# LuletterSoul/RP-Style-Transfer

Hardware: AMD Instinct MI355X
Metric: stylized images/sec at 512×512, 1/2/4/8 MI355X; % HBM roofline (higher is better)
Workload: dtype fp32

## Files before the change

include/rpst.h:

```cpp
#ifndef RPST_H_
#define RPST_H_

#include <stddef.h>
#include <stdint.h>

#ifdef __cplusplus
extern "C" {
#endif

typedef void* rpst_stream_t;

#define RPST_OK 0
#define RPST_EINVAL (-1)
#define RPST_EHIP (-2)
#define RPST_EWORKSPACE (-3)

#define RPST_PAD_ZERO 0
#define RPST_PAD_REFLECT 1
#define RPST_IN_NONE 0
#define RPST_IN_MAXPOOL2 1
#define RPST_IN_UPSAMPLE2 2
#define RPST_IN_ADD_UPSAMPLE2 3
#define RPST_IN_ADAIN 4
#define RPST_IN_ADD_ADAIN 5
// ... 95 lines not shown
                          size_t workspace_bytes, rpst_stream_t stream);
int rpst_ld4_fuse(const float* y, const float* fine, const float* coarse,
                  const float* params_fine, const float* params_coarse, float* out, int N,
                  int Ca, int hidden, int H, int W, int h, int w, rpst_stream_t stream);

int rpst_conv2d_skip_adain(const float* stylized, const float* content, const float* params,
                           const float* packed_weight, const float* bias, float* out, int N,
                           int Cin, int H, int W, int Cout, int ksize, int pad_mode, int relu,
                           rpst_stream_t stream);

int64_t rpst_conv2d_grid_threads(int N, int Cin, int Hs, int Ws, int Cout, int ksize,
                                 int in_op);

#define RPST_CONV_DIRECT 0
#define RPST_CONV_WINOGRAD 1
#define RPST_CONV_WINOGRAD4 2
#define RPST_CONV_NARROW 3
int rpst_conv2d_algorithm(int Cout, int Cin, int Hs, int Ws, int ksize, int in_op);

int rpst_conv2d_set_precise(int on);

int rpst_conv2d_set_quarter(int mode);
int rpst_conv2d_quarter(int Cout, int Cin, int Hs, int Ws, int ksize, int in_op);

int rpst_maxpool2x2_ceil(const float* in, float* out, int N, int C, int H, int W,
                         rpst_stream_t stream);
int rpst_upsample_nearest2x(const float* in, float* out, int N, int C, int H, int W,
                            rpst_stream_t stream);
int rpst_add_upsample_nearest2x(const float* a, const float* b, float* out, int N, int C, int H,
                                int W, rpst_stream_t stream);

size_t rpst_sanet_attention_workspace_size(int B, int HW);
size_t rpst_sanet_attention_workspace_size_c(int B, int C, int HW);
int rpst_sanet_attention(const float* F, const float* G, const float* H, float* O, int B,
                         int C, int HW, void* workspace, size_t workspace_bytes,
                         rpst_stream_t stream);

size_t rpst_cosine_affinity_workspace_size(int B, int C, int HW);
int rpst_cosine_affinity(const float* content, const float* style, float* out, int B, int C,
                         int HW, void* workspace, size_t workspace_bytes, rpst_stream_t stream);

size_t rpst_aea_clamp_workspace_size(int B, int HW, int hidden);
int rpst_aea_clamp(const float* x, const float* fx, const float* w1, const float* b1,
                   const float* w2, const float* b2, int hidden, int mode, float scale,
                   float from, float interval, float* out_fx, float* out_clamp, int B, int HW,
                   void* workspace, size_t workspace_bytes, rpst_stream_t stream);
// ... 134 lines not shown
```

rp-style-transfer_amd/csrc/rpst_conv.h:

```cpp
#pragma once

#include "rpst_common.h"

namespace rpst {

constexpr int kTW = 32;

struct ConvArgs {
  const float* in;
  const float* aux;
  const float* aux2;
  const float* wpk;
  const float* bias;
  const float* res;
  float* out;
  int N, Cin, Hs, Ws, H, W, Cout, Cout_pad, nchunks;
  int tiles_x, tiles_y, co_tiles;
  int pad, relu;
  int persist;
  int cosplit;
  float2* stat_part;
  int stat_P;
  int64_t wstride;
  const float* btab;
  int skip_from;
  const float* in2;
  int in2_from;
  const float* mask;
  int pool_out;
};

struct ConvMode {
  int precise;
  int quarter;
  int algo;
  bool narrow;
  int narrow_rpt;
};

struct ConvTiling {
  int64_t blocks;
  int nth;
  int stat_nt, stat_wn, stat_tw;
  bool stat_t;
};

__device__ __forceinline__ const float* conv_in_img(const ConvArgs& a, int n, int64_t per) {
  return (a.in2_from > 0 && n >= a.in2_from) ? a.in2 + (int64_t)(n - a.in2_from) * per
                                             : a.in + (int64_t)n * per;
}

template <int KS>
struct ConvK {
  static constexpr int CK = (KS == 3) ? 8 : 16;
  static constexpr int TAPS = KS * KS;
  static constexpr int KCH = TAPS * CK;
};
// ... 222 lines not shown
```

rp-style-transfer_amd/csrc/rpst_conv.hip:

```cpp
#include "rpst_conv.h"

#include <cstdlib>
#include <cstring>

namespace rpst {

template <int KS, int BM, int TH, int WM, int WN, int INOP, int NTH, int CKK, bool DB,
          bool GATED = false>
__global__ __launch_bounds__(NTH, 2) void conv_mfma_kernel(ConvArgs a) {
  using K = ConvK<KS>;
  constexpr int PCK = K::CK, TAPS = K::TAPS;
  constexpr int CK = CKK, KCH = TAPS * CK;
  static_assert(PCK % CK == 0, "kernel chunk must divide the packing chunk");
  constexpr int OFF = (KS == 3) ? 1 : 0;
  constexpr int PH = TH + KS - 1, PW = kTW + KS - 1;
  constexpr int WTM = BM / WM;
  constexpr int MT = WTM / 32;
  constexpr int NT = TH / WN;
  static_assert(WM * WN == NTH / kWave, "one wave per sub-tile");
  static_assert(MT >= 1 && NT >= 1 && (CK % 2) == 0, "tile");
  constexpr int NW4 = KCH * BM / 4;
  constexpr int WLD = (NW4 + NTH - 1) / NTH;
  constexpr bool WFULL = (NW4 % NTH) == 0;
  constexpr int GROUPS = NTH / 32;
// ... 532 lines not shown
  a.tiles_x = (a.W + kTW - 1) / kTW;
  a.tiles_y = (a.H + th - 1) / th;
  a.co_tiles = a.Cout_pad / bm;
  a.stat_P = a.tiles_x * a.tiles_y * wn;
  return {(int64_t)a.tiles_x * a.tiles_y * a.N * a.co_tiles, 256, th / wn, wn, kTW, false};
}

static int narrow_rpt(int Cout, const ConvMode& m) {
  return Cout <= 4 && m.narrow_rpt != 2 ? 4 : 2;
}
static ConvTiling narrow_tiling(ConvArgs& a, int rpt) {
  const int rows = 4 * rpt;
  a.Cout_pad = pad_cout(a.Cout);
  a.nchunks = (a.Cin + ConvK<3>::CK - 1) / ConvK<3>::CK;
  a.tiles_x = (a.W + kNrTW - 1) / kNrTW;
  a.tiles_y = (a.H + rows - 1) / rows;
  a.co_tiles = 1;
  a.stat_P = 0;
  return {(int64_t)a.tiles_x * a.tiles_y * a.N, 256, 0, 0, kNrTW, false};
}

static thread_local int t_conv_precise = 0;
static thread_local int t_conv_quarter = -1;

static ConvMode conv_mode() {
  ConvMode m{};
  m.precise = t_conv_precise;
  const char* e = getenv("RPST_W4Q");
  const int q = t_conv_quarter >= 0 ? t_conv_quarter : ((e && *e) ? atoi(e) : 1);
  m.quarter = q == 2 ? 2 : q != 0;
  e = getenv("RPST_CONV_ALGO");
  m.algo = -1;
  if (e && e[0] == 'd') m.algo = RPST_CONV_DIRECT;
  else if (e && !strcmp(e, "winograd")) m.algo = RPST_CONV_WINOGRAD;
  else if (e && !strcmp(e, "winograd4")) m.algo = RPST_CONV_WINOGRAD4;
  e = getenv("RPST_CONV_NARROW");
  m.narrow = !(e && *e && atoi(e) == 0);
  e = getenv("RPST_CONV_NARROW_RPT");
  m.narrow_rpt = (e && *e && atoi(e) == 2) ? 2 : 0;
  return m;
}

static int conv_algo(int Cout, int Cin, int Hs, int Ws, int ksize, int in_op, const ConvMode& m) {
  if (ksize != 3) return RPST_CONV_DIRECT;
  const bool w4 = wino4_supports(in_op) && wino4_fits(1, Cin, Hs, Ws, in_op);
  const bool nr = (in_op == RPST_IN_NONE || (in_op == RPST_IN_ADD_ADAIN && Cout <= 4)) &&
                  narrow_shape(Cin, Cout) && m.narrow;
  if (m.algo == RPST_CONV_DIRECT) return nr ? RPST_CONV_NARROW : RPST_CONV_DIRECT;
  if (m.algo == RPST_CONV_WINOGRAD) return RPST_CONV_WINOGRAD;
  if (m.algo == RPST_CONV_WINOGRAD4) return w4 ? RPST_CONV_WINOGRAD4 : RPST_CONV_WINOGRAD;
  if (nr) return RPST_CONV_NARROW;
  if (Cin <= 4 && w4 && m.precise != 1) return RPST_CONV_WINOGRAD4;
  if (Cin < 16) return RPST_CONV_DIRECT;
// ... 38 lines not shown
  int rpt;
  size_t wofs;
  bool tall;
  ConvTiling t;
};

static ConvPlan conv_plan(ConvArgs& a, int ksize, int in_op, const ConvMode& m, ConvNeeds need) {
  ConvPlan p{};
  p.op = in_op;
  p.algo = conv_algo(a.Cout, a.Cin, a.Hs, a.Ws, ksize, in_op, m);
  if (p.algo == RPST_CONV_NARROW) {
    p.rpt = narrow_rpt(a.Cout, m);
    p.t = narrow_tiling(a, p.rpt);
    if (need.stats || a.N > 65535 || a.tiles_y > 65535) p.algo = RPST_CONV_DIRECT;
  }
  if (need.residual && (p.algo == RPST_CONV_WINOGRAD || p.algo == RPST_CONV_WINOGRAD4))
    p.algo = RPST_CONV_DIRECT;
  if (p.algo == RPST_CONV_WINOGRAD4) {
    p.fold = need.fold && !need.stats && a.H >= 2 && a.W >= 2;
    if (p.fold) p.op = RPST_IN_NONE;
    p.quarter = wino4q_applies(a.Cin, a.Cout, p.op, m);
    p.wofs = direct_packed_floats(a.Cout, a.Cin, ksize) + wino_packed_floats(a.Cout, a.Cin) +
             (p.quarter ? wino4_packed_floats(a.Cout, a.Cin) : 0);
    p.t = p.quarter ? wino4q_tiling(a) : wino4_tiling(a);
  } else if (p.algo == RPST_CONV_WINOGRAD) {
    p.wofs = direct_packed_floats(a.Cout, a.Cin, ksize);
    p.t = wino_tiling(a, in_op);
  } else if (p.algo == RPST_CONV_DIRECT) {
    p.tall = need.gated && need.stats && direct_bm(a.Cout) != 128;
    p.t = direct_tiling(a, ksize, in_op, p.tall);
  }
  return p;
}

template <class F>
static size_t max_over_modes(ConvMode m, F bytes) {
  size_t best = 0;
  for (m.precise = 0; m.precise < 3; ++m.precise)
    for (m.quarter = 0; m.quarter < 3; ++m.quarter) {
      const size_t b = bytes(m);
      best = b > best ? b : best;
    }
  return best;
}

}
// ... 11 lines not shown

static ConvPlan query_plan(int N, int Cin, int Hs, int Ws, int Cout, int ksize, int in_op) {
  ConvArgs a = conv_shape(N, Cin, Hs, Ws, Cout, in_op);
  return conv_plan(a, ksize, in_op, conv_mode(), {});
}

extern "C" int64_t rpst_conv2d_grid_threads(int N, int Cin, int Hs, int Ws, int Cout,
                                            int ksize, int in_op) {
  if (N <= 0 || Cin <= 0 || Hs <= 0 || Ws <= 0 || Cout <= 0 || (ksize != 1 && ksize != 3))
    return 0;
  const ConvTiling t = query_plan(N, Cin, Hs, Ws, Cout, ksize, in_op).t;
  return t.blocks * t.nth;
}

extern "C" int rpst_conv2d_set_precise(int on) {
  const int old = t_conv_precise;
  t_conv_precise = on == 2 ? 2 : on != 0;
  return old;
}

extern "C" int rpst_conv2d_set_quarter(int mode) {
  const int old = t_conv_quarter;
  t_conv_quarter = mode < 0 ? -1 : (mode > 2 ? 2 : mode);
  return old;
}

extern "C" int rpst_conv2d_algorithm(int Cout, int Cin, int Hs, int Ws, int ksize, int in_op) {
  return query_plan(1, Cin, Hs, Ws, Cout, ksize, in_op).algo;
}

extern "C" int rpst_conv2d_quarter(int Cout, int Cin, int Hs, int Ws, int ksize, int in_op) {
  return query_plan(1, Cin, Hs, Ws, Cout, ksize, in_op).quarter ? 1 : 0;
}

extern "C" int rpst_conv2d_pack(const float* weight, float* packed, int Cout, int Cin,
                                int ksize, rpst_stream_t stream) {
  RPST_REQUIRE(weight && packed, "conv2d_pack: null pointer");
  RPST_REQUIRE(Cout > 0 && Cin > 0, "conv2d_pack: bad channels");
  RPST_REQUIRE(ksize == 1 || ksize == 3, "conv2d_pack: ksize must be 1 or 3, got %d", ksize);
  const int64_t total = (int64_t)direct_packed_floats(Cout, Cin, ksize);
  const int threads = 256;
  conv_pack_kernel<<<(unsigned)((total + threads - 1) / threads), threads, 0,
                     as_stream(stream)>>>(weight, packed, Cout, Cin, ksize, ck_of(ksize),
                                          pad_cout(Cout), total);
  if (int e = launch_status("conv_pack_kernel")) return e;
  if (ksize == 3) {
// ... 522 lines not shown
```

rp-style-transfer_amd/csrc/rpst_wino4q.hip:

```cpp
#include "rpst_conv.h"

#include <type_traits>

#ifndef RPST_W4Q_DBG
#define RPST_W4Q_DBG 0
#endif

namespace rpst {
namespace {

template <int PAD>
__device__ __forceinline__ void q_mfma(floatx4& acc, float a, float b) {
  if constexpr (PAD)
    asm volatile("s_nop 1\n\tv_mfma_f32_16x16x4_f32 %0, %1, %2, %0" : "+v"(acc) : "v"(a), "v"(b));
  else
    asm volatile("v_mfma_f32_16x16x4_f32 %0, %1, %2, %0" : "+v"(acc) : "v"(a), "v"(b));
}
__device__ __forceinline__ unsigned q_lds_addr(const float* p) {
  return (unsigned)(uintptr_t)(const __attribute__((address_space(3))) float*)p;
}
template <int OFF>
__device__ __forceinline__ void q_dma16(__amdgpu_buffer_rsrc_t r, unsigned m0, unsigned voff,
                                        int soff) {
  asm volatile("s_mov_b32 m0, %0\n\ts_nop 0\n\tbuffer_load_dwordx4 %1, %2, %3 offen offset:%4 lds"
// ... 24 lines not shown
    u2 = fmaf(4.f, d1, fmaf(-5.f, d3, d5));
  }
}

}

constexpr int kQCo = 64;
constexpr int kQTH = 8, kQTW = 64;
constexpr int kQXO = 4;
constexpr int kQPS = 72;
constexpr int kQCS = 768;
constexpr int kQWS = 9216;
constexpr int kQPAT = 4 * kQCS;
constexpr int kQNTH = 512;
constexpr int kQMaxCo = 512;
constexpr int kQWPI = 5;
constexpr int kQWide = 2, kQSlow = 6;
constexpr int kQDMA4 = 3, kQDMA = 12;
constexpr int kQRP = kQPS / 4;
constexpr int kQXS = 4 * 3 * 3 * 64 * 2;
constexpr int kQWG0 = 0;
constexpr int kQPG = 5;
constexpr int kQAhead = 3;
static_assert(10 * kQRP <= kQDMA4 * 64 && kQDMA4 * 256 <= kQCS, "16-B pieces in a channel");
static_assert(10 * kQPS <= kQDMA * 64 && kQDMA * 64 <= kQCS, "4-B pieces in a channel");
static_assert(2 * kQWide >= kQDMA4 && 2 * kQSlow >= kQDMA && 8 * kQWPI >= 36, "coverage");
static_assert(2 * kQXS <= kQWS, "the exchange fits a weight stage");
static_assert((2 * kQWS + 4 * kQPAT) * 4 + 1024 + kQSlow * kQNTH * 4 + 9 * kQMaxCo * 4 <= 163840,
              "LDS");

template <typename TW>
__global__ void wino4q_pack_kernel(const TW* __restrict__ w, float* __restrict__ pk, int Cout,
                                   int Cin, int K4, int64_t per, int64_t total, int64_t sco,
                                   int64_t sci, int64_t stap) {
  int64_t t = (int64_t)blockIdx.x * blockDim.x + threadIdx.x;
  if (t >= total) return;
  const int64_t img = t / per;
  pk += img * per;
  w += img * (int64_t)Cout * Cin * 9;
  t -= img * per;
  const int cb = (int)(t & 3);
  int64_t r = t >> 2;
  const int l = (int)(r & 63);
  r >>= 6;
  const int p = (int)(r % 9);
  r /= 9;
// ... 53 lines not shown
  const int ci = ks * 4 + (l >> 4);
  const int64_t nc = (int64_t)N * Cin, i = (int64_t)n * Cin + (ci < Cin ? ci : 0);
  const float sc = ci < Cin ? aux[3 * nc + i] / aux[2 * nc + i] : 0.f;
  const float4 v = pk[u];
  out[t] = make_float4(v.x * sc, v.y * sc, v.z * sc, v.w * sc);
}

int wino4q_fold_w(const float* pk, float* out, const float* aux, int N, int Cout, int Cin,
                  hipStream_t st) {
  const int64_t per4 = (int64_t)wino4q_packed_floats(Cout, Cin) / 4, n4 = (int64_t)N * per4;
  wino4q_fold_w_kernel<<<(unsigned)((n4 + 255) / 256), 256, 0, st>>>(
      reinterpret_cast<const float4*>(pk), reinterpret_cast<float4*>(out), aux, N, Cin,
      (Cin + 3) / 4, per4);
  return launch_status("wino4q_fold_w_kernel");
}

bool wino4q_applies(int Cin, int Cout, int in_op, const ConvMode& m) {
  const int min_cin = m.quarter == 2 ? 16 : 128;
  return m.quarter && m.precise != 2 && (in_op == RPST_IN_NONE || in_op == RPST_IN_UPSAMPLE2) &&
         Cout >= 64 && Cout <= kQMaxCo &&
         Cin >= min_cin && Cin % 16 == 0;
}

ConvTiling wino4q_tiling(ConvArgs& a) {
  a.Cout_pad = (a.Cout + kQCo - 1) / kQCo * kQCo;
  a.nchunks = (a.Cin + 3) / 4;
  a.tiles_x = (a.W + kQTW - 1) / kQTW;
  a.tiles_y = (a.H + kQTH - 1) / kQTH;
  a.co_tiles = a.Cout_pad / kQCo;
  a.stat_P = a.tiles_x * a.tiles_y * 2;
  a.cosplit = 1;
  return {(int64_t)a.tiles_x * a.tiles_y * a.N, kQNTH, 4, kQTH / 4, kQTW, true};
}

struct QEpi {
  int W, H, Cout, gy0, gx0, rows, n, sidx;
  bool vec, full, bst, edge, store, pool;
  float inv, slope;
  unsigned voff[4];
  float* out;
  float* oimg;
  unsigned obytes;
  const float* btab;
  float2* statp;
  int statP;
};

__device__ __forceinline__ QEpi q_epi_ctx(int wr, int tn) {
  const KArgs L = late_args();
  QEpi e;
  e.W = L->W;
  e.H = L->H;
  e.Cout = L->Cout;
  e.slope = L->relu == RPST_ACT_RELU ? 0.f : (L->relu == RPST_ACT_LRELU ? 0.2f : 1.f);
  int btx, bty;
  w4_tile((int)blockIdx.x / L->cosplit, L->tiles_x, L->tiles_y, btx, bty, e.n);
  const int bx0 = btx * kQTW;
  e.gy0 = bty * kQTH + 4 * wr;
  e.gx0 = bx0 + 4 * tn;
  e.vec = (e.W & 3) == 0 && e.gx0 + 3 < e.W;
  e.rows = max(0, min(4, e.H - e.gy0));
  const int cols = max(0, min(kQTW, e.W - bx0));
  e.inv = e.rows * cols > 0 ? __builtin_amdgcn_rcpf((float)(e.rows * cols)) : 0.f;
  e.full = e.rows == 4 && bx0 + kQTW <= e.W;
  e.edge = e.gy0 == 0 || e.gy0 + 4 >= e.H || bx0 == 0 || bx0 + kQTW >= e.W;
  e.out = L->out;
  const int64_t plane = (int64_t)e.H * e.W;
  e.pool = L->pool_out != 0;
  e.bst = !e.pool && (e.W & 3) == 0 && (int64_t)e.Cout * plane * 4 < (1LL << 31);
  e.oimg = e.out + (int64_t)e.n * e.Cout * plane;
  const bool keep = L->skip_from <= 0 || e.n < L->skip_from;
  e.obytes = keep ? (unsigned)(e.Cout * plane * 4) : 0u;
  e.store = keep;
#pragma unroll
  for (int yy = 0; yy < 4; ++yy)
    e.voff[yy] = (yy < e.rows && e.gx0 < e.W) ? (unsigned)(((e.gy0 + yy) * e.W + e.gx0) * 4)
                                             : 0x80000000u;
  e.btab = L->btab;
  e.statp = L->stat_part;
// ... 120 lines not shown
  }
}

template <int INOP, bool STATS, bool BTAB, bool RELU>
__global__ __launch_bounds__(kQNTH, 1) void wino4q_mfma_kernel(ConvArgs a) {
  __shared__ __attribute__((aligned(16))) float ws0[kQWS];
  __shared__ __attribute__((aligned(16))) float ws1[kQWS];
  __shared__ __attribute__((aligned(16))) float ps0[kQPAT];
  __shared__ __attribute__((aligned(16))) float ps1[kQPAT];
  __shared__ __attribute__((aligned(16))) float ps2[kQPAT];
  __shared__ __attribute__((aligned(16))) float ps3[kQPAT];
  __shared__ __attribute__((aligned(16))) float dummy[256];
  __shared__ unsigned poffs[kQSlow][kQNTH];
  __shared__ float btl[BTAB ? 9 * kQMaxCo : kQMaxCo];

  const int wave = __builtin_amdgcn_readfirstlane((int)threadIdx.x >> 6);
  const int lane = threadIdx.x & 63;
  const int k = lane >> 4, tn = lane & 15, wr = wave >> 2;

  int bid = (int)blockIdx.x;
  const int cog = bid % a.cosplit;
  bid /= a.cosplit;
  const int nct = a.co_tiles / a.cosplit, ct0 = cog * nct;
  int tx, ty, n;
  w4_tile(bid, a.tiles_x, a.tiles_y, tx, ty, n);
  const int K4 = a.nchunks, G = nct * K4;
  const int y0 = ty * kQTH, x0 = tx * kQTW;

  {
    const int nb = BTAB ? 9 * a.Cout : a.Cout;
    const float* src = BTAB ? a.btab + (int64_t)n * nb : a.bias;
    for (int i = threadIdx.x; i < nb; i += kQNTH) btl[i] = src ? src[i] : 0.f;
  }
  constexpr bool up = INOP == RPST_IN_UPSAMPLE2;
  const unsigned in_plane = up ? (unsigned)(a.Hs * a.Ws) : (unsigned)(a.H * a.W);
  const unsigned oob = a.Cin * in_plane * 4u;
  const float* in_img = conv_in_img(a, n, (int64_t)a.Cin * in_plane);
  const unsigned wbytes = (unsigned)(nct * K4 * kQWS) * 4u;
  const float* w_img = a.wpk + (int64_t)n * a.wstride + (int64_t)ct0 * K4 * kQWS;

  const int hf = wave & 1;
  const bool zp = a.pad == RPST_PAD_ZERO;
  const int rs = up ? a.Ws : a.W;
  const bool w4a = (a.W & 3) == 0;
  const bool wide = !up && ((x0 >= 1 && x0 + kQTW < a.W) || (w4a && x0 + kQTW <= a.W));
  const bool fixL = wide && w4a && !zp && x0 == 0;
  const bool fixR = wide && w4a && !zp && x0 + kQTW == a.W;
  unsigned poff[kQSlow];
  const int tid = threadIdx.x;
  if (wide) {
#pragma unroll
    for (int i = 0; i < kQWide; ++i) {
      const int p = kQWide * hf + i;
      const int f = 64 * p + lane, row = min(f / kQRP, 9), j = f - (f / kQRP) * kQRP;
      int y = y0 - 1 + row;
      const int xs = x0 - kQXO + 4 * j;
      const bool okx = !w4a || (xs >= 0 && xs + 3 < a.W);
      const bool ok = p < kQDMA4 && f < 10 * kQRP && resolve_bf(y, a.H, zp) && okx;
      poff[i] = ok ? ((unsigned)(y * rs) + (unsigned)xs) * 4u : oob;
    }
#pragma unroll
    for (int i = kQWide; i < kQSlow; ++i) poff[i] = oob;
  } else {
#pragma unroll
    for (int i = 0; i < kQSlow; ++i) {
      const int p = kQSlow * hf + i;
      const int f = 64 * p + lane;
      const int row = min(f / kQPS, 9), col = f - (f / kQPS) * kQPS;
      int y = y0 - 1 + row, x = x0 - kQXO + col;
      const bool oky = resolve_bf(y, a.H, zp), okx = resolve_bf(x, a.W, zp);
      const bool ok = p < kQDMA && col >= kQXO - 1 && col < kQXO + 1 + kQTW &&
                      f < 10 * kQPS && oky && okx;
      poff[i] = ok ? ((unsigned)((up ? y >> 1 : y) * rs) + (unsigned)(up ? x >> 1 : x)) * 4u : oob;
    }
  }
#pragma unroll
  for (int i = 0; i < kQSlow; ++i) poffs[i][tid] = poff[i];

  constexpr int DBG = RPST_W4Q_DBG;
  const int wl = wave * 4096;
  const bool real4 = wave < 4;
  const int w4 = 32768 + wave * 1024;
  const unsigned dummy_a = q_lds_addr(dummy);
  int wso = wl;
  auto issue_w = [&](bool live, unsigned stg, auto Ic) {
    constexpr int I = decltype(Ic)::value;
    if (DBG & 2) return;
    if constexpr (I < 4) {
      q_dma16<1024 * I>(rsrc_or_zero(w_img, wbytes, live), stg + wl, lane * 16, wso);
    } else {
      q_dma16<0>(rsrc_or_zero(w_img, wbytes, live && real4), real4 ? stg + w4 : dummy_a,
                 lane * 16, wso + (w4 - wl));
    }
  };
  const unsigned pstep = 4u * in_plane * 4u;
  const int pbase = (int)((unsigned)(wave >> 1) * in_plane * 4u);
  const bool h1 = (wave & 1) != 0;
  const int pl = (wave >> 1) * (kQCS * 4) + (h1 ? (wide ? 2048 : kQSlow * 256) : 0);
  int pso = pbase;
  auto issue_p = [&](auto WIDEc, bool live, unsigned stg) {
    constexpr bool WIDE = decltype(WIDEc)::value;
    if (DBG & 1) return;
    const auto r = rsrc_or_zero(in_img, oob, live);
    const unsigned xs = stg + launder(pl);
    if constexpr (WIDE) {
      q_dma16<0>(r, xs, poffs[0][tid], pso);
      q_dma16<0>(r, h1 ? dummy_a : xs + 1024, poffs[1][tid], pso);
    } else {
#pragma unroll
      for (int i = 0; i < kQSlow; ++i) q_dma4(r, xs + 256 * i, poffs[i][tid], pso);
    }
    pso += (int)pstep;
  };
  const bool bst_all = !a.pool_out && (a.W & 3) == 0 &&
                       (int64_t)a.Cout * a.H * a.W * 4 < (1LL << 31);
  bool post_epi = false;
  auto wait_ring = [&](bool first) {
    if (DBG & 128) return;
    if (first && post_epi && bst_all) {
      if (wide) asm volatile("s_waitcnt vmcnt(18)" ::: "memory");
      else asm volatile("s_waitcnt vmcnt(22)" ::: "memory");
    } else if (wide) {
      asm volatile("s_waitcnt vmcnt(2)" ::: "memory");
    } else {
      asm volatile("s_waitcnt vmcnt(6)" ::: "memory");
    }
    if (first) post_epi = false;
  };

  auto fix_halo = [&](float* stg) {
    if ((wave == 0 && fixL) || (wave == 1 && fixR)) {
      int l = lane;
      asm volatile("" : "+v"(l));
      if (l < 40) {
        const int ch = l / 10, row = l - 10 * ch;
        float* rp = stg + ch * kQCS + row * kQPS;
        if (wave == 0) rp[kQXO - 1] = rp[kQXO + 1];
        else rp[kQXO + kQTW] = rp[kQXO + kQTW - 2];
      }
    }
  };
  auto prologue = [&](auto WIDEc) {
    issue_p(WIDEc, true, q_lds_addr(ps0));
    issue_p(WIDEc, true, q_lds_addr(ps1));
    issue_w(true, q_lds_addr(ws0), std::integral_constant<int, 0>{});
    issue_w(true, q_lds_addr(ws0), std::integral_constant<int, 1>{});
    issue_w(true, q_lds_addr(ws0), std::integral_constant<int, 2>{});
    issue_w(true, q_lds_addr(ws0), std::integral_constant<int, 3>{});
    issue_w(true, q_lds_addr(ws0), std::integral_constant<int, 4>{});
    issue_p(WIDEc, true, q_lds_addr(ps2));
    issue_p(WIDEc, true, q_lds_addr(ps3));
  };
  if (wide) prologue(std::true_type{});
  else prologue(std::false_type{});
  wait_ring(false);
  q_lds_barrier();
  if (fixL || fixR) {
    fix_halo(ps0);
    fix_halo(ps1);
    q_lds_barrier();
  }

  auto body = [&](auto Qc) {
    constexpr int Q = decltype(Qc)::value, QR = Q >> 1, QC = Q & 1;
    floatx4 acc[9][4];
#pragma unroll
    for (int p = 0; p < 9; ++p)
#pragma unroll
      for (int cb = 0; cb < 4; ++cb) acc[p][cb] = floatx4{0.f, 0.f, 0.f, 0.f};
    const int roff = k * kQCS + (4 * wr + QR) * kQPS + 4 * tn;
    auto read_row = [&](const float* stg, int rr, float (&d)[8]) {
      const float* rp = stg + roff + rr * kQPS;
      floatx4 u = *reinterpret_cast<const floatx4*>(rp + 4);
      const float e = QC ? rp[8] : rp[3];
      asm("" : "+v"(u));
      d[0] = QC ? 0.f : e; d[1] = u[0]; d[2] = u[1]; d[3] = u[2]; d[4] = u[3];
      d[5] = QC ? e : 0.f; d[6] = 0.f; d[7] = 0.f;
    };
    auto col_pass = [&](const float (&d)[8], float (&u)[3]) {
      if (DBG & 8) {
        u[0] = d[0]; u[1] = d[1]; u[2] = d[2];
        return;
      }
      q_bt3<QC>(d[0], d[1], d[2], d[3], d[4], d[5], u[0], u[1], u[2]);
    };
    auto row_pass = [&](const float (&u)[5][3], int j, float (&v)[9]) {
      if (DBG & 8) {
        v[j] = u[0][j]; v[3 + j] = u[2][j]; v[6 + j] = u[4][j];
        return;
      }
      if constexpr (QR == 0)
        q_bt3<0>(u[0][j], u[1][j], u[2][j], u[3][j], u[4][j], 0.f, v[j], v[3 + j], v[6 + j]);
      else
        q_bt3<1>(0.f, u[0][j], u[1][j], u[2][j], u[3][j], u[4][j], v[j], v[3 + j], v[6 + j]);
    };
    float V[9];
    {
      float u[5][3];
#pragma unroll
      for (int rr = 0; rr < 5; ++rr) {
        float d[8];
        read_row(ps0, rr, d);
        col_pass(d, u[rr]);
      }
#pragma unroll
      for (int j = 0; j < 3; ++j) row_pass(u, j, V);
    }

    const int woff = Q * 9 * 256 + lane * 4;
    int x = 0;
    auto step = [&](float* wsx, float* psn, float* wsn, float* psx, float* pfx, int ks,
                    bool first) {
      wait_ring(first);
      const bool wlive = x + 1 < G, plive = x + 4 < G;
      wso += kQWS * 4;
      if (first && ks + 4 == K4) pso = pbase;
      const unsigned wsn_a = q_lds_addr(wsn), psx_a = q_lds_addr(psx);
      if (DBG & 16) asm volatile("s_waitcnt lgkmcnt(0)" ::: "memory");
      else q_lds_barrier();
      constexpr int ord[9] = {0, 3, 6, 1, 4, 7, 2, 5, 8};
      constexpr int kA = kQAhead;
      float4 w4[9];
#pragma unroll
      for (int q = 0; q < kA; ++q)
        w4[ord[q]] = *reinterpret_cast<const float4*>(wsx + woff + ord[q] * 256);
      float d[8];
      read_row(psn, 0, d);
      float u[5][3];
#pragma unroll
      for (int q = 0; q < 9; ++q) {
// ... 3 lines not shown
        q_mfma<1>(acc[p][0], w4[p].x, V[p]);
        q_mfma<0>(acc[p][1], w4[p].y, V[p]);
        q_mfma<0>(acc[p][2], w4[p].z, V[p]);
        q_mfma<0>(acc[p][3], w4[p].w, V[p]);
        if (q == kQWG0) issue_w(wlive, wsn_a, std::integral_constant<int, 0>{});
        if (q == kQWG0 + 1) issue_w(wlive, wsn_a, std::integral_constant<int, 1>{});
        if (q == kQWG0 + 2) issue_w(wlive, wsn_a, std::integral_constant<int, 2>{});
        if (q == kQWG0 + 3) issue_w(wlive, wsn_a, std::integral_constant<int, 3>{});
        if (q == kQWG0 + 4) issue_w(wlive, wsn_a, std::integral_constant<int, 4>{});
        if (q == kQPG) {
          if (wide) issue_p(std::true_type{}, plive, psx_a);
          else issue_p(std::false_type{}, plive, psx_a);
        }
        if (q < 5) {
          col_pass(d, u[q]);
          if (q + 1 < 5) read_row(psn, q + 1, d);
        }
        if (q == 5 || q == 6 || q == 8) row_pass(u, q == 8 ? 2 : q - 5, V);
        if (q == 7) fix_halo(pfx);
      }
      ++x;
    };

    auto epilogue = [&](int ctile) {
      if (DBG & 32) {
        float t = 0.f;
#pragma unroll
        for (int p = 0; p < 9; ++p)
#pragma unroll
          for (int cb = 0; cb < 4; ++cb) t += acc[p][cb][0];
        if (t == 1.2345f) late_args()->out[threadIdx.x] = t;
#pragma unroll
        for (int p = 0; p < 9; ++p)
#pragma unroll
          for (int cb = 0; cb < 4; ++cb) acc[p][cb] = floatx4{0.f, 0.f, 0.f, 0.f};
        return;
      }
      q_lds_barrier();
      asm volatile("s_nop 7\n\ts_nop 4" : "+v"(acc[0][0]), "+v"(acc[0][1]), "+v"(acc[0][2]),
                   "+v"(acc[0][3]), "+v"(acc[1][0]), "+v"(acc[1][1]), "+v"(acc[1][2]),
                   "+v"(acc[1][3]), "+v"(acc[2][0]), "+v"(acc[2][1]), "+v"(acc[2][2]),
                   "+v"(acc[2][3]), "+v"(acc[3][0]), "+v"(acc[3][1]), "+v"(acc[3][2]),
                   "+v"(acc[3][3]), "+v"(acc[4][0]), "+v"(acc[4][1]));
      asm volatile("" : "+v"(acc[4][2]), "+v"(acc[4][3]), "+v"(acc[5][0]), "+v"(acc[5][1]),
                   "+v"(acc[5][2]), "+v"(acc[5][3]), "+v"(acc[6][0]), "+v"(acc[6][1]),
                   "+v"(acc[6][2]), "+v"(acc[6][3]), "+v"(acc[7][0]), "+v"(acc[7][1]),
                   "+v"(acc[7][2]), "+v"(acc[7][3]), "+v"(acc[8][0]), "+v"(acc[8][1]),
                   "+v"(acc[8][2]), "+v"(acc[8][3]));
      const int co0 = ctile * kQCo + 16 * Q + 4 * k;
#pragma unroll
      for (int rp = 0; rp < 2; ++rp) {
        float P[2][6][4];
#pragma unroll
        for (int pt = 0; pt < 3; ++pt) {
          float* xb = ws1 + wr * kQXS;
#pragma unroll
          for (int dq = 0; dq < 4; ++dq) {
            if (dq == Q || (DBG & 4)) continue;
            const int slot = (Q - dq - 1) & 3;
#pragma unroll
            for (int j = 0; j < 3; ++j)
// ... 8 lines not shown
            for (int j = 0; j < 3; ++j) {
              float2 v;
              if (s == Q || (DBG & 4)) {
                const int src = (DBG & 4) ? s : Q;
                v = make_float2(acc[3 * pt + j][src][2 * rp], acc[3 * pt + j][src][2 * rp + 1]);
              } else {
                v = *reinterpret_cast<const float2*>(
                    xb + (((Q * 3 + ((s - Q - 1) & 3)) * 3 + j) * 64 + lane) * 2);
              }
              m[0][s >> 1][3 * (s & 1) + j] = v.x;
              m[1][s >> 1][3 * (s & 1) + j] = v.y;
            }
          }
#pragma unroll
          for (int e2 = 0; e2 < 2; ++e2) {
            at6(m[e2][0], P[e2][pt]);
            at6(m[e2][1], P[e2][3 + pt]);
          }
          if (!(DBG & 4) && (rp == 0 || pt < 2)) q_lds_barrier();
        }
#pragma unroll
        for (int e2 = 0; e2 < 2; ++e2) {
          const int r = 2 * rp + e2;
          QEpi e = q_epi_ctx(wr, tn);
          e.btab = btl;
          float bias = 0.f;
          {
            const int co = co0 + r;
            if (co < e.Cout) bias = BTAB ? btl[co * 9 + 4] : btl[co];
          }
#pragma unroll
          for (int x = 0; x < 4; ++x) P[e2][1][x] += bias;
          float Y[16];
#pragma unroll
          for (int x = 0; x < 4; ++x) {
            float c6[6], y[4];
#pragma unroll
            for (int I = 0; I < 6; ++I) c6[I] = P[e2][I][x];
            at6(c6, y);
#pragma unroll
            for (int yy = 0; yy < 4; ++yy) Y[yy * 4 + x] = y[yy];
          }
          q_finish<STATS, BTAB, RELU>(e, co0 + r, Y, tn);
        }
      }
#pragma unroll
      for (int p = 0; p < 9; ++p)
#pragma unroll
        for (int cb = 0; cb < 4; ++cb) acc[p][cb] = floatx4{0.f, 0.f, 0.f, 0.f};
    };

    int ks = 0, ct = ct0;
    for (int g = 0; g < G; g += 4) {
      step(ws0, ps1, ws1, ps0, ps2, ks, true);
      step(ws1, ps2, ws0, ps1, ps3, ks + 1, false);
      step(ws0, ps3, ws1, ps2, ps0, ks + 2, false);
      step(ws1, ps0, ws0, ps3, ps1, ks + 3, false);
      ks += 4;
      if (ks == K4) {
        epilogue(ct);
        post_epi = true;
        ks = 0;
        ++ct;
      }
    }
  };
  switch (wave & 3) {
    case 0: body(std::integral_constant<int, 0>{}); break;
    case 1: body(std::integral_constant<int, 1>{}); break;
    case 2: body(std::integral_constant<int, 2>{}); break;
    default: body(std::integral_constant<int, 3>{}); break;
  }
  asm volatile("s_waitcnt vmcnt(0)" ::: "memory");
}

int wino4q_launch(ConvArgs& a, int in_op, hipStream_t st) {
  RPST_REQUIRE(in_op == RPST_IN_NONE || in_op == RPST_IN_UPSAMPLE2,
               "conv2d: winograd4 (quarter) does not support in_op %d", in_op);
  const ConvTiling t = wino4q_tiling(a);
  RPST_REQUIRE((int64_t)a.co_tiles * a.nchunks * kQWS * 4 < (1LL << 31),
               "conv2d: winograd4 weight image exceeds 2 GiB");
  RPST_REQUIRE(t.blocks <= 0x7fffffffLL, "conv2d: grid too large");
  const unsigned nb = (unsigned)t.blocks;
  const bool stats = a.stat_part != nullptr, btab = a.btab != nullptr;
  RPST_REQUIRE(!btab || in_op == RPST_IN_NONE, "conv2d: winograd4 bias table with a loader op");
  RPST_REQUIRE(!(stats && btab), "conv2d: winograd4 folded bias with statistics");
#define RPST_W4Q_GO(OP, S, B)                                                  \
  do {                                                                         \
    if (a.relu == RPST_ACT_RELU)                                               \
      wino4q_mfma_kernel<OP, S, B, true><<<nb, kQNTH, 0, st>>>(a);             \
    else                                                                       \
      wino4q_mfma_kernel<OP, S, B, false><<<nb, kQNTH, 0, st>>>(a);            \
  } while (0)
  if (in_op == RPST_IN_UPSAMPLE2) {
    if (stats) RPST_W4Q_GO(RPST_IN_UPSAMPLE2, true, false);
    else RPST_W4Q_GO(RPST_IN_UPSAMPLE2, false, false);
  } else {
// ... 10 lines not shown
```

rp-style-transfer_amd/rpst/_lib.py:

```python
from __future__ import annotations

import ctypes
import os
import threading

_HERE = os.path.dirname(os.path.abspath(__file__))
LIB_PATH = os.environ.get("RPST_LIB", os.path.join(os.path.dirname(_HERE), "csrc", "librpst.so"))

_c_float_p = ctypes.c_void_p
_P = ctypes.c_void_p
_I = ctypes.c_int
_I64 = ctypes.c_int64
_F = ctypes.c_float
_D = ctypes.c_double
_SZ = ctypes.c_size_t

SIGNATURES = {
    "rpst_version": (_I, []),
    "rpst_last_error": (ctypes.c_char_p, []),
    "rpst_calc_mean_std": (_I, [_P, _P, _P, _I, _I, _I64, _F, _P]),
    "rpst_adain_workspace_size": (_SZ, [_I, _I]),
    "rpst_adain": (_I, [_P, _P, _P, _I, _I, _I64, _F, _P, _SZ, _P]),
    "rpst_mean_variance_norm": (_I, [_P, _P, _I, _I, _I64, _F, _P, _SZ, _P]),
    "rpst_segment_plan": (_I, [_P, _P, _I, _I64, _I64, _P, _P]),
    "rpst_masked_adain_workspace_size": (_SZ, [_I, _I]),
    "rpst_masked_adain_params": (_I, [_P, _P, _P, _P, _P, _I, _I, _I64, _I64, _F, _P, _P, _SZ,
                                      _P]),
    "rpst_masked_adain_apply": (_I, [_P, _P, _P, _P, _P, _I, _I, _I64, _P]),
    "rpst_conv2d_packed_size": (_SZ, [_I, _I, _I]),
    "rpst_conv2d_pack": (_I, [_P, _P, _I, _I, _I, _P]),
    "rpst_conv2d_grid_threads": (_I64, [_I, _I, _I, _I, _I, _I, _I]),
    "rpst_conv2d_algorithm": (_I, [_I, _I, _I, _I, _I, _I]),
    "rpst_conv2d_set_precise": (_I, [_I]),
    "rpst_conv2d_set_quarter": (_I, [_I]),
    "rpst_conv2d_quarter": (_I, [_I, _I, _I, _I, _I, _I]),
    "rpst_conv2d_stats_workspace_size": (_SZ, [_I, _I, _I, _I, _I, _I, _I]),
    "rpst_conv2d_stats": (_I, [_P, _P, _P, _P, _P, _P, _I, _I, _I, _I, _I, _I, _I, _I, _I,
                               _P, _P, _F, _P, _SZ, _P]),
    "rpst_conv2d_stats_store": (_I, [_P, _P, _P, _P, _P, _P, _I, _I, _I, _I, _I, _I, _I, _I,
                                     _I, _P, _P, _F, _I, _P, _SZ, _P]),
    "rpst_conv2d": (_I, [_P, _P, _P, _P, _P, _P, _I, _I, _I, _I, _I, _I, _I, _I, _I, _P]),
    "rpst_conv2d_pool": (_I, [_P, _P, _P, _P, _P, _I, _I, _I, _I, _I, _I, _I, _I, _I, _P]),
    "rpst_conv2d_masked": (_I, [_P, _P, _P, _P, _P, _I, _I, _I, _I, _I, _I, _I, _P]),
    "rpst_conv2d_pair": (_I, [_P, _P, _I, _P, _P, _P, _I, _I, _I, _I, _I, _I, _I, _I, _P]),
    "rpst_conv2d_workspace_size": (_SZ, [_I, _I, _I, _I, _I, _I, _I]),
    "rpst_conv2d_ws": (_I, [_P, _P, _P, _P, _P, _P, _I, _I, _I, _I, _I, _I, _I, _I, _I,
                            _P, _SZ, _P]),
    "rpst_conv2d_skip_adain": (_I, [_P, _P, _P, _P, _P, _P, _I, _I, _I, _I, _I, _I, _I, _I, _P]),
    "rpst_se_gate": (_I, [_P, _P, _P, _P, _P, _P, _I, _I, _I, _P]),
    "rpst_conv2d_gated_workspace_size": (_SZ, [_I, _I, _I, _I, _I, _I]),
    "rpst_conv2d_gated": (_I, [_P, _P, _P, _P, _P, _P, _I, _I, _I, _I, _I, _I, _P, _P, _F, _P,
                               _SZ, _P]),
    "rpst_conv7_packed_size": (_SZ, [_I, _I]),
    "rpst_conv7_pack": (_I, [_P, _P, _I, _I, _P]),
    "rpst_conv7": (_I, [_P, _P, _P, _P, _P, _I, _I, _I, _I, _I, _I, _I, _I, _I, _P]),
    "rpst_nearest_index_table": (_I, [_I, _I, _P]),
    "rpst_resize_nearest": (_I, [_P, _P, _I, _I, _I, _I, _I, _I, _I, _I, _P]),
# ... 109 lines not shown
```

Before: 570.1.

## Process multiple spatial tiles per block in quarter-Winograd conv with prefetched next tile

The quarter-precision Winograd-4 conv kernel now has each block walk several consecutive output tiles instead of one. The next tile's input and weight DMA prologue is issued during the current tile's epilogue, so global loads overlap the output writes. By default a heuristic picks 2 tiles per block when the reduction is short and there are enough tiles, otherwise 1; an env var or setter can override it. This cuts launch and prologue cost and hides tile-start latency, at the price of fewer blocks (less parallelism) and more complex synchronisation through hand-tuned vmcnt waits. A debug timestamp path is also added behind a compile flag.

```diff
diff --git a/include/rpst.h b/include/rpst.h
--- a/include/rpst.h
+++ b/include/rpst.h
@@ -141,6 +141,8 @@
 
 int rpst_conv2d_set_quarter(int mode);
 int rpst_conv2d_quarter(int Cout, int Cin, int Hs, int Ws, int ksize, int in_op);
+
+int rpst_conv2d_set_tiles(int tiles);
 
 int rpst_maxpool2x2_ceil(const float* in, float* out, int N, int C, int H, int W,
                          rpst_stream_t stream);
diff --git a/rp-style-transfer_amd/csrc/rpst_conv.h b/rp-style-transfer_amd/csrc/rpst_conv.h
--- a/rp-style-transfer_amd/csrc/rpst_conv.h
+++ b/rp-style-transfer_amd/csrc/rpst_conv.h
@@ -28,11 +28,13 @@
   int in2_from;
   const float* mask;
   int pool_out;
+  int wtiles;
 };
 
 struct ConvMode {
   int precise;
   int quarter;
+  int tiles;
   int algo;
   bool narrow;
   int narrow_rpt;
diff --git a/rp-style-transfer_amd/csrc/rpst_conv.hip b/rp-style-transfer_amd/csrc/rpst_conv.hip
--- a/rp-style-transfer_amd/csrc/rpst_conv.hip
+++ b/rp-style-transfer_amd/csrc/rpst_conv.hip
@@ -578,6 +578,7 @@
 
 static thread_local int t_conv_precise = 0;
 static thread_local int t_conv_quarter = -1;
+static thread_local int t_conv_tiles = -1;
 
 static ConvMode conv_mode() {
   ConvMode m{};
@@ -585,6 +586,8 @@
   const char* e = getenv("RPST_W4Q");
   const int q = t_conv_quarter >= 0 ? t_conv_quarter : ((e && *e) ? atoi(e) : 1);
   m.quarter = q == 2 ? 2 : q != 0;
+  e = getenv("RPST_W4Q_TILES");
+  m.tiles = t_conv_tiles > 0 ? t_conv_tiles : ((e && *e) ? atoi(e) : -1);
   e = getenv("RPST_CONV_ALGO");
   m.algo = -1;
   if (e && e[0] == 'd') m.algo = RPST_CONV_DIRECT;
@@ -669,6 +672,7 @@
     p.quarter = wino4q_applies(a.Cin, a.Cout, p.op, m);
     p.wofs = direct_packed_floats(a.Cout, a.Cin, ksize) + wino_packed_floats(a.Cout, a.Cin) +
              (p.quarter ? wino4_packed_floats(a.Cout, a.Cin) : 0);
+    a.wtiles = m.tiles;
     p.t = p.quarter ? wino4q_tiling(a) : wino4_tiling(a);
   } else if (p.algo == RPST_CONV_WINOGRAD) {
     p.wofs = direct_packed_floats(a.Cout, a.Cin, ksize);
@@ -726,6 +730,12 @@
 extern "C" int rpst_conv2d_set_quarter(int mode) {
   const int old = t_conv_quarter;
   t_conv_quarter = mode < 0 ? -1 : (mode > 2 ? 2 : mode);
+  return old;
+}
+
+extern "C" int rpst_conv2d_set_tiles(int tiles) {
+  const int old = t_conv_tiles;
+  t_conv_tiles = tiles <= 0 ? -1 : tiles;
   return old;
 }
 
diff --git a/rp-style-transfer_amd/csrc/rpst_wino4q.hip b/rp-style-transfer_amd/csrc/rpst_wino4q.hip
--- a/rp-style-transfer_amd/csrc/rpst_wino4q.hip
+++ b/rp-style-transfer_amd/csrc/rpst_wino4q.hip
@@ -70,6 +70,11 @@
 constexpr int kQWG0 = 0;
 constexpr int kQPG = 5;
 constexpr int kQAhead = 3;
+constexpr int kQMaxTiles = 64;
+#if RPST_W4Q_DBG & 256
+constexpr int kQStampBlocks = 1 << 16;
+__device__ unsigned long long g_w4q_stamps[kQStampBlocks * 8];
+#endif
 static_assert(10 * kQRP <= kQDMA4 * 64 && kQDMA4 * 256 <= kQCS, "16-B pieces in a channel");
 static_assert(10 * kQPS <= kQDMA * 64 && kQDMA * 64 <= kQCS, "4-B pieces in a channel");
 static_assert(2 * kQWide >= kQDMA4 && 2 * kQSlow >= kQDMA && 8 * kQWPI >= 36, "coverage");
@@ -169,6 +174,11 @@
          Cin >= min_cin && Cin % 16 == 0;
 }
 
+static int wino4q_tiles_rule(int steps, int64_t tiles) {
+  const int t = steps <= 32 ? 2 : 1;
+  return tiles >= (int64_t)2 * 256 * t ? t : 1;
+}
+
 ConvTiling wino4q_tiling(ConvArgs& a) {
   a.Cout_pad = (a.Cout + kQCo - 1) / kQCo * kQCo;
   a.nchunks = (a.Cin + 3) / 4;
@@ -177,7 +187,10 @@
   a.co_tiles = a.Cout_pad / kQCo;
   a.stat_P = a.tiles_x * a.tiles_y * 2;
   a.cosplit = 1;
-  return {(int64_t)a.tiles_x * a.tiles_y * a.N, kQNTH, 4, kQTH / 4, kQTW, true};
+  const int64_t tiles = (int64_t)a.tiles_x * a.tiles_y * a.N;
+  if (a.wtiles <= 0) a.wtiles = wino4q_tiles_rule(a.co_tiles * a.nchunks, tiles);
+  a.wtiles = a.wtiles > kQMaxTiles ? kQMaxTiles : a.wtiles;
+  return {(tiles + a.wtiles - 1) / a.wtiles, kQNTH, 4, kQTH / 4, kQTW, true};
 }
 
 struct QEpi {
@@ -193,7 +206,7 @@
   int statP;
 };
 
-__device__ __forceinline__ QEpi q_epi_ctx(int wr, int tn) {
+__device__ __forceinline__ QEpi q_epi_ctx(int wr, int tn, int tile) {
   const KArgs L = late_args();
   QEpi e;
   e.W = L->W;
@@ -201,7 +214,7 @@
   e.Cout = L->Cout;
   e.slope = L->relu == RPST_ACT_RELU ? 0.f : (L->relu == RPST_ACT_LRELU ? 0.2f : 1.f);
   int btx, bty;
-  w4_tile((int)blockIdx.x / L->cosplit, L->tiles_x, L->tiles_y, btx, bty, e.n);
+  w4_tile(tile, L->tiles_x, L->tiles_y, btx, bty, e.n);
   const int bx0 = btx * kQTW;
   e.gy0 = bty * kQTH + 4 * wr;
   e.gx0 = bx0 + 4 * tn;
@@ -368,67 +381,94 @@
   const int cog = bid % a.cosplit;
   bid /= a.cosplit;
   const int nct = a.co_tiles / a.cosplit, ct0 = cog * nct;
-  int tx, ty, n;
-  w4_tile(bid, a.tiles_x, a.tiles_y, tx, ty, n);
   const int K4 = a.nchunks, G = nct * K4;
-  const int y0 = ty * kQTH, x0 = tx * kQTW;
-
-  {
-    const int nb = BTAB ? 9 * a.Cout : a.Cout;
-    const float* src = BTAB ? a.btab + (int64_t)n * nb : a.bias;
+  int tile = bid * a.wtiles;
+  const int ntile = min(a.wtiles, a.tiles_x * a.tiles_y * a.N - tile);
+
+  auto fill_btl = [&](int t, auto L) __attribute__((always_inline)) {
+    const int n = t / (L->tiles_x * L->tiles_y);
+    const int nb = BTAB ? 9 * L->Cout : L->Cout;
+    const float* src = BTAB ? L->btab + (int64_t)n * nb : L->bias;
     for (int i = threadIdx.x; i < nb; i += kQNTH) btl[i] = src ? src[i] : 0.f;
-  }
+  };
   constexpr bool up = INOP == RPST_IN_UPSAMPLE2;
   const unsigned in_plane = up ? (unsigned)(a.Hs * a.Ws) : (unsigned)(a.H * a.W);
   const unsigned oob = a.Cin * in_plane * 4u;
-  const float* in_img = conv_in_img(a, n, (int64_t)a.Cin * in_plane);
   const unsigned wbytes = (unsigned)(nct * K4 * kQWS) * 4u;
-  const float* w_img = a.wpk + (int64_t)n * a.wstride + (int64_t)ct0 * K4 * kQWS;
 
   const int hf = wave & 1;
-  const bool zp = a.pad == RPST_PAD_ZERO;
-  const int rs = up ? a.Ws : a.W;
-  const bool w4a = (a.W & 3) == 0;
-  const bool wide = !up && ((x0 >= 1 && x0 + kQTW < a.W) || (w4a && x0 + kQTW <= a.W));
-  const bool fixL = wide && w4a && !zp && x0 == 0;
-  const bool fixR = wide && w4a && !zp && x0 + kQTW == a.W;
-  unsigned poff[kQSlow];
   const int tid = threadIdx.x;
-  if (wide) {
-#pragma unroll
-    for (int i = 0; i < kQWide; ++i) {
-      const int p = kQWide * hf + i;
-      const int f = 64 * p + lane, row = min(f / kQRP, 9), j = f - (f / kQRP) * kQRP;
-      int y = y0 - 1 + row;
-      const int xs = x0 - kQXO + 4 * j;
-      const bool okx = !w4a || (xs >= 0 && xs + 3 < a.W);
-      const bool ok = p < kQDMA4 && f < 10 * kQRP && resolve_bf(y, a.H, zp) && okx;
-      poff[i] = ok ? ((unsigned)(y * rs) + (unsigned)xs) * 4u : oob;
-    }
-#pragma unroll
-    for (int i = kQWide; i < kQSlow; ++i) poff[i] = oob;
-  } else {
-#pragma unroll
-    for (int i = 0; i < kQSlow; ++i) {
-      const int p = kQSlow * hf + i;
-      const int f = 64 * p + lane;
-      const int row = min(f / kQPS, 9), col = f - (f / kQPS) * kQPS;
-      int y = y0 - 1 + row, x = x0 - kQXO + col;
-      const bool oky = resolve_bf(y, a.H, zp), okx = resolve_bf(x, a.W, zp);
-      const bool ok = p < kQDMA && col >= kQXO - 1 && col < kQXO + 1 + kQTW &&
-                      f < 10 * kQPS && oky && okx;
-      poff[i] = ok ? ((unsigned)((up ? y >> 1 : y) * rs) + (unsigned)(up ? x >> 1 : x)) * 4u : oob;
-    }
-  }
-#pragma unroll
-  for (int i = 0; i < kQSlow; ++i) poffs[i][tid] = poff[i];
+  const int wl = wave * 4096;
+  const unsigned pstep = 4u * in_plane * 4u;
+  const int pbase = (int)((unsigned)(wave >> 1) * in_plane * 4u);
+  const bool h1 = (wave & 1) != 0;
+  int wso = wl, pso = pbase, pl = 0;
+  bool wide = false, fixL = false, fixR = false;
+  const float* in_img = nullptr;
+  const float* w_img = nullptr;
+  auto set_tile = [&](int t, auto L) __attribute__((always_inline)) {
+    const int W = L->W, H = L->H;
+    int ln = lane;
+    asm volatile("" : "+v"(ln));
+    t = launder(t);
+    int tx, ty, n;
+    w4_tile(t, L->tiles_x, L->tiles_y, tx, ty, n);
+    const int y0 = ty * kQTH, x0 = tx * kQTW;
+    const bool zp = L->pad == RPST_PAD_ZERO;
+    const int rs = up ? L->Ws : W;
+    const bool w4a = (W & 3) == 0;
+    wide = !up && (w4a ? x0 + kQTW <= W : (x0 >= 1 && x0 + kQTW + kQXO <= W));
+    fixL = wide && w4a && !zp && x0 == 0;
+    fixR = wide && w4a && !zp && x0 + kQTW == W;
+    const int64_t per = (int64_t)L->Cin * in_plane;
+    in_img = (L->in2_from > 0 && n >= L->in2_from) ? L->in2 + (int64_t)(n - L->in2_from) * per
+                                                   : L->in + (int64_t)n * per;
+    w_img = L->wpk + (int64_t)n * L->wstride + (int64_t)ct0 * K4 * kQWS;
+    wso = wl;
+    pso = pbase;
+    pl = (wave >> 1) * (kQCS * 4) + (h1 ? (wide ? 2048 : kQSlow * 256) : 0);
+    unsigned poff[kQSlow];
+    if (wide) {
+#pragma unroll
+      for (int i = 0; i < kQWide; ++i) {
+        const int p = kQWide * hf + i;
+        const int f = 64 * p + ln, row = min(f / kQRP, 9), j = f - (f / kQRP) * kQRP;
+        int y = y0 - 1 + row;
+        const int xs = x0 - kQXO + 4 * j;
+        const bool okx = !w4a || (xs >= 0 && xs + 3 < W);
+        const bool ok = p < kQDMA4 && f < 10 * kQRP && resolve_bf(y, H, zp) && okx;
+        poff[i] = ok ? ((unsigned)(y * rs) + (unsigned)xs) * 4u : oob;
+      }
+#pragma unroll
+      for (int i = kQWide; i < kQSlow; ++i) poff[i] = oob;
+    } else {
+#pragma unroll
+      for (int i = 0; i < kQSlow; ++i) {
+        const int p = kQSlow * hf + i;
+        const int f = 64 * p + ln;
+        const int row = min(f / kQPS, 9), col = f - (f / kQPS) * kQPS;
+        int y = y0 - 1 + row, x = x0 - kQXO + col;
+        const bool oky = resolve_bf(y, H, zp), okx = resolve_bf(x, W, zp);
+        const bool ok = p < kQDMA && col >= kQXO - 1 && col < kQXO + 1 + kQTW &&
+                        f < 10 * kQPS && oky && okx;
+        poff[i] = ok ? ((unsigned)((up ? y >> 1 : y) * rs) + (unsigned)(up ? x >> 1 : x)) * 4u : oob;
+      }
+    }
+#pragma unroll
+    for (int i = 0; i < kQSlow; ++i) poffs[i][tid] = poff[i];
+  };
 
   constexpr int DBG = RPST_W4Q_DBG;
-  const int wl = wave * 4096;
+#if RPST_W4Q_DBG & 256
+  unsigned long long stamps[5] = {0, 0, 0, 0, 0};
+  const unsigned long long real0 = __builtin_amdgcn_s_memrealtime();
+  auto q_stamp = [&](int i) { stamps[i] = __builtin_amdgcn_s_memtime(); };
+#else
+  auto q_stamp = [](int) {};
+#endif
   const bool real4 = wave < 4;
   const int w4 = 32768 + wave * 1024;
   const unsigned dummy_a = q_lds_addr(dummy);
-  int wso = wl;
   auto issue_w = [&](bool live, unsigned stg, auto Ic) {
     constexpr int I = decltype(Ic)::value;
     if (DBG & 2) return;
@@ -439,11 +479,6 @@
                  lane * 16, wso + (w4 - wl));
     }
   };
-  const unsigned pstep = 4u * in_plane * 4u;
-  const int pbase = (int)((unsigned)(wave >> 1) * in_plane * 4u);
-  const bool h1 = (wave & 1) != 0;
-  const int pl = (wave >> 1) * (kQCS * 4) + (h1 ? (wide ? 2048 : kQSlow * 256) : 0);
-  int pso = pbase;
   auto issue_p = [&](auto WIDEc, bool live, unsigned stg) {
     constexpr bool WIDE = decltype(WIDEc)::value;
     if (DBG & 1) return;
@@ -473,6 +508,17 @@
     }
     if (first) post_epi = false;
   };
+  auto wait_tile = [&](bool hoisted) __attribute__((always_inline)) {
+    if (DBG & 128) return;
+    if (hoisted && bst_all) {
+      if (wide) asm volatile("s_waitcnt vmcnt(18)" ::: "memory");
+      else asm volatile("s_waitcnt vmcnt(22)" ::: "memory");
+    } else if (wide) {
+      asm volatile("s_waitcnt vmcnt(2)" ::: "memory");
+    } else {
+      asm volatile("s_waitcnt vmcnt(6)" ::: "memory");
+    }
+  };
 
   auto fix_halo = [&](float* stg) {
     if ((wave == 0 && fixL) || (wave == 1 && fixR)) {
@@ -486,7 +532,7 @@
       }
     }
   };
-  auto prologue = [&](auto WIDEc) {
+  auto prologue = [&](auto WIDEc) __attribute__((always_inline)) {
     issue_p(WIDEc, true, q_lds_addr(ps0));
     issue_p(WIDEc, true, q_lds_addr(ps1));
     issue_w(true, q_lds_addr(ws0), std::integral_constant<int, 0>{});
@@ -497,15 +543,26 @@
     issue_p(WIDEc, true, q_lds_addr(ps2));
     issue_p(WIDEc, true, q_lds_addr(ps3));
   };
-  if (wide) prologue(std::true_type{});
-  else prologue(std::false_type{});
-  wait_ring(false);
-  q_lds_barrier();
-  if (fixL || fixR) {
-    fix_halo(ps0);
-    fix_halo(ps1);
+  auto start_tile = [&](int t, auto L) __attribute__((always_inline)) {
+    set_tile(t, L);
+    if (wide) prologue(std::true_type{});
+    else prologue(std::false_type{});
+  };
+  auto open_tile = [&](bool hoisted) __attribute__((always_inline)) {
+    wait_tile(hoisted);
     q_lds_barrier();
-  }
+    if (fixL || fixR) {
+      fix_halo(ps0);
+      fix_halo(ps1);
+      q_lds_barrier();
+    }
+  };
+  q_stamp(0);
+  constexpr bool dma_first = BTAB && !(DBG & 512);
+  if (!dma_first) fill_btl(tile, &a);
+  start_tile(tile, &a);
+  if (dma_first) fill_btl(tile, &a);
+  open_tile(false);
 
   auto body = [&](auto Qc) {
     constexpr int Q = decltype(Qc)::value, QR = Q >> 1, QC = Q & 1;
@@ -541,7 +598,7 @@
         q_bt3<1>(0.f, u[0][j], u[1][j], u[2][j], u[3][j], u[4][j], v[j], v[3 + j], v[6 + j]);
     };
     float V[9];
-    {
+    auto form_v0 = [&]() __attribute__((always_inline)) {
       float u[5][3];
 #pragma unroll
       for (int rr = 0; rr < 5; ++rr) {
@@ -551,7 +608,9 @@
       }
 #pragma unroll
       for (int j = 0; j < 3; ++j) row_pass(u, j, V);
-    }
+    };
+    form_v0();
+    q_stamp(1);
 
     const int woff = Q * 9 * 256 + lane * 4;
     int x = 0;
@@ -601,8 +660,13 @@
       ++x;
     };
 
-    auto epilogue = [&](int ctile) {
+    auto epilogue = [&](int ctile, bool hoist) __attribute__((always_inline)) {
+      if (hoist) asm volatile("s_waitcnt vmcnt(0)" ::: "memory");
       if (DBG & 32) {
+        if (hoist) {
+          q_lds_barrier();
+          start_tile(tile + 1, late_args());
+        }
         float t = 0.f;
 #pragma unroll
         for (int p = 0; p < 9; ++p)
@@ -616,6 +680,7 @@
         return;
       }
       q_lds_barrier();
+      if (hoist) start_tile(tile + 1, late_args());
       asm volatile("s_nop 7\n\ts_nop 4" : "+v"(acc[0][0]), "+v"(acc[0][1]), "+v"(acc[0][2]),
                    "+v"(acc[0][3]), "+v"(acc[1][0]), "+v"(acc[1][1]), "+v"(acc[1][2]),
                    "+v"(acc[1][3]), "+v"(acc[2][0]), "+v"(acc[2][1]), "+v"(acc[2][2]),
@@ -670,7 +735,7 @@
 #pragma unroll
         for (int e2 = 0; e2 < 2; ++e2) {
           const int r = 2 * rp + e2;
-          QEpi e = q_epi_ctx(wr, tn);
+          QEpi e = q_epi_ctx(wr, tn, tile);
           e.btab = btl;
           float bias = 0.f;
           {
@@ -699,17 +764,41 @@
     };
 
     int ks = 0, ct = ct0;
-    for (int g = 0; g < G; g += 4) {
+    const int Gall = G * ntile;
+    for (int g = 0; g < Gall; g += 4) {
       step(ws0, ps1, ws1, ps0, ps2, ks, true);
       step(ws1, ps2, ws0, ps1, ps3, ks + 1, false);
       step(ws0, ps3, ws1, ps2, ps0, ks + 2, false);
       step(ws1, ps0, ws0, ps3, ps1, ks + 3, false);
       ks += 4;
       if (ks == K4) {
-        epilogue(ct);
+        const bool last = ct + 1 == ct0 + nct;
+        const bool more = last && g + 4 < Gall;
+        bool hoist = more;
+        if constexpr (BTAB) {
+          const int per = late_args()->tiles_x * late_args()->tiles_y;
+          hoist = more && (tile + 1) / per == tile / per;
+        }
+        if (last && !more) q_stamp(2);
+        epilogue(ct, hoist);
+        if (last && !more) q_stamp(3);
         post_epi = true;
         ks = 0;
         ++ct;
+        if (more) {
+          if (!hoist) {
+            asm volatile("s_waitcnt vmcnt(0)" ::: "memory");
+            q_lds_barrier();
+            fill_btl(tile + 1, late_args());
+            start_tile(tile + 1, late_args());
+            post_epi = false;
+          }
+          ++tile;
+          ct = ct0;
+          x = 0;
+          open_tile(hoist);
+          form_v0();
+        }
       }
     }
   };
@@ -720,7 +809,29 @@
     default: body(std::integral_constant<int, 3>{}); break;
   }
   asm volatile("s_waitcnt vmcnt(0)" ::: "memory");
-}
+#if RPST_W4Q_DBG & 256
+  q_stamp(4);
+  if (threadIdx.x == 0 && blockIdx.x < kQStampBlocks) {
+    unsigned long long* s = g_w4q_stamps + (size_t)blockIdx.x * 8;
+#pragma unroll
+    for (int i = 0; i < 5; ++i) s[i] = stamps[i];
+    s[5] = (unsigned)__builtin_amdgcn_s_getreg((31 << 11) | 4) |
+           (unsigned long long)(unsigned)__builtin_amdgcn_s_getreg((31 << 11) | 20) << 32;
+    s[6] = real0;
+    s[7] = __builtin_amdgcn_s_memrealtime();
+  }
+#endif
+}
+
+#if RPST_W4Q_DBG & 256
+}
+extern "C" int rpst_w4q_dbg_stamps(unsigned long long* host, size_t blocks) {
+  if (blocks > (size_t)rpst::kQStampBlocks) blocks = rpst::kQStampBlocks;
+  return (int)hipMemcpyFromSymbol(host, HIP_SYMBOL(rpst::g_w4q_stamps), blocks * 64, 0,
+                                  hipMemcpyDeviceToHost);
+}
+namespace rpst {
+#endif
 
 int wino4q_launch(ConvArgs& a, int in_op, hipStream_t st) {
   RPST_REQUIRE(in_op == RPST_IN_NONE || in_op == RPST_IN_UPSAMPLE2,
diff --git a/rp-style-transfer_amd/rpst/_lib.py b/rp-style-transfer_amd/rpst/_lib.py
--- a/rp-style-transfer_amd/rpst/_lib.py
+++ b/rp-style-transfer_amd/rpst/_lib.py
@@ -33,6 +33,7 @@
     "rpst_conv2d_algorithm": (_I, [_I, _I, _I, _I, _I, _I]),
     "rpst_conv2d_set_precise": (_I, [_I]),
     "rpst_conv2d_set_quarter": (_I, [_I]),
+    "rpst_conv2d_set_tiles": (_I, [_I]),
     "rpst_conv2d_quarter": (_I, [_I, _I, _I, _I, _I, _I]),
     "rpst_conv2d_stats_workspace_size": (_SZ, [_I, _I, _I, _I, _I, _I, _I]),
     "rpst_conv2d_stats": (_I, [_P, _P, _P, _P, _P, _P, _I, _I, _I, _I, _I, _I, _I, _I, _I,
```

Result: no change. 572.2 (median of 6 runs) (+0.4%).
